# DerryHub/BEVFormer_tensorrt

Hardware: AMD Instinct MI355X
Metric: frames/sec BEVFormer-base bs=1 fp16 end-to-end on MI355X (re-hosted model, random weights, synthetic 6-camera frames) (higher is better)
Workload: dtype f16

## Files before the change

bevformer_tensorrt_amd/csrc/mdconv.h:

```cpp
#ifndef BEVOPS_MDCONV_H_
#define BEVOPS_MDCONV_H_
#include <type_traits>

#include "common.h"

namespace bevops {
enum DcnPath {
  kDcnAuto = 0,
  kDcnLds,
  kDcnStaged,
  kDcnGemm
};

struct DcnVariant {
  int id;
  DcnPath f16, s8;
  int f16_threads;
  bool no_tail, wide;
};
extern thread_local DcnVariant g_dcn_variant;

namespace {

typedef _Float16 f16x8 __attribute__((ext_vector_type(8)));
typedef float f32x16 __attribute__((ext_vector_type(16)));

struct ConvDims {
  int B, Cin, H, W, Cout, Kh, Kw, sh, sw, ph, pw, dh, dw, G, DG, Ho, Wo;
};

template <typename T> __device__ __forceinline__ float tof(T v);
template <> __device__ __forceinline__ float tof<float>(float v) { return v; }
template <> __device__ __forceinline__ float tof<__half>(__half v) { return __half2float(v); }
template <typename T> __device__ __forceinline__ T fromf(float v);
template <> __device__ __forceinline__ float fromf<float>(float v) { return v; }
template <> __device__ __forceinline__ __half fromf<__half>(float v) { return __float2half_rn(v); }

template <typename T>
__global__ __launch_bounds__(256) void nchw_to_nhwc_kernel(const T *__restrict__ in,
                                                           T *__restrict__ out, int C, int HW, int flip = 0) {
  __shared__ T tile[32][33];
  const int b = blockIdx.z;
  const int p0 = blockIdx.x * 32, c0 = blockIdx.y * 32;
  const int tx = threadIdx.x & 31, ty = threadIdx.x >> 5;
  const T *ib = in + (size_t)b * C * HW;
  T *ob = out + (size_t)b * C * HW;
#pragma unroll
  for (int r = 0; r < 32; r += 8) {
    const int c = c0 + ty + r, p = p0 + tx;
    if (c < C && p < HW) {
      if constexpr (sizeof(T) == 1) tile[ty + r][tx] = (T)(ib[(size_t)c * HW + p] ^ (T)flip);
      else tile[ty + r][tx] = ib[(size_t)c * HW + p];
    }
  }
  __syncthreads();
#pragma unroll
  for (int r = 0; r < 32; r += 8) {
    const int p = p0 + ty + r, c = c0 + tx;
    if (c < C && p < HW) ob[(size_t)p * C + c] = tile[tx][ty + r];
  }
}

template <typename T>
__global__ __launch_bounds__(256) void repack_weight_kernel(const T *__restrict__ w,
                                                            T *__restrict__ wt, int Cout,
                                                            int cin_g, int KK, int row_stride) {
  const size_t i = (size_t)blockIdx.x * 256 + threadIdx.x;
  const size_t total = (size_t)Cout * cin_g * KK;
  if (i >= total) return;
  const int ci = (int)(i % cin_g);
  const int t = (int)((i / cin_g) % KK);
  const size_t co = i / ((size_t)cin_g * KK);
  wt[co * row_stride + (size_t)t * cin_g + ci] = w[(co * cin_g + ci) * KK + t];
}

constexpr int kBM = 128, kBN = 128, kBK = 32, kLd = kBK + 8;

struct GemmEpi {
  int HoWo, Cout, co0;
};

constexpr int kFM = 256, kFN = 64, kFK = 64, kFLd = kFK + 8;

constexpr int kGA = kFM * kFK * 2;
template <int WN> struct Glds {
  static constexpr int kN = 32 * WN;
  static constexpr int kThreads = 256 * WN;
  static constexpr int kB = kN * kFK * 2;
  static constexpr int kLds = 2 * (kGA + kB);
  static constexpr int kPieces = 32 / (4 * WN);
};

typedef unsigned u32x4_t __attribute__((ext_vector_type(4)));
__device__ __forceinline__ unsigned swz8(unsigned r) { return (r ^ (r >> 3)) & 7u; }

struct TailPlan {
  int tail_tiles, split, main_tiles;
  float *partial;
  int out_nhwc, relu;
  int om_channels;
};

inline size_t align256(size_t x) { return (x + 255) & ~size_t(255); }

inline bool make_dims(ConvDims &d, int B, int Cin, int H, int W, int Cout, int Kh, int Kw, int sh, int sw,
               int ph, int pw, int dh, int dw, int G, int DG) {
  if (B <= 0 || Cin <= 0 || H <= 0 || W <= 0 || Cout <= 0 || Kh <= 0 || Kw <= 0 || sh <= 0 ||
      sw <= 0 || ph < 0 || pw < 0 || dh <= 0 || dw <= 0 || G <= 0 || DG <= 0)
    return false;
  if (Cin % G || Cout % G || Cin % DG) return false;
  const int Ho = (H + 2 * ph - (dh * (Kh - 1) + 1)) / sh + 1;
  const int Wo = (W + 2 * pw - (dw * (Kw - 1) + 1)) / sw + 1;
  if (Ho <= 0 || Wo <= 0) return false;
  d = ConvDims{B, Cin, H, W, Cout, Kh, Kw, sh, sw, ph, pw, dh, dw, G, DG, Ho, Wo};
  return true;
}

struct WsLayout {
  size_t xt, wt, col, total;
};
inline size_t kpad(const ConvDims &d, size_t es) {
  const size_t kg = (size_t)(d.Cin / d.G) * d.Kh * d.Kw;
  return es == 1 ? ((kg + 15) & ~size_t(15)) : kg;
}
inline WsLayout ws_layout(const ConvDims &d, size_t es) {
  WsLayout w;
  const size_t kp = kpad(d, es);
  w.xt = 0;
  w.wt = align256((size_t)d.B * d.Cin * d.H * d.W * es);
  w.col = w.wt + align256((size_t)d.Cout * kp * es);
  w.total = w.col + align256((size_t)d.B * d.Ho * d.Wo * d.G * kp * es);
  return w;
}

struct DcnCall {
  ConvDims d;
  int dtype;
  const void *input, *offset, *mask, *weight, *bias;
  void *output;
  bool packed;
  bool nhwc;
  bool relu;
  bool exact;
  int om_channels;
  float s_in, s_off, s_mask, s_w, s_out;
  void *workspace;
  size_t workspace_bytes;
  hipStream_t stream;
};

inline DcnCall dcn_call(int dtype, const void *input, const void *offset, const void *mask, const void *weight,
                        const void *bias, void *output, void *workspace, size_t workspace_bytes, int B, int Cin, int H,
                        int W, int Cout, int Kh, int Kw, int sh, int sw, int ph, int pw, int dh, int dw, int G, int DG,
                        void *stream) {
  DcnCall c{};
  (void)make_dims(c.d, B, Cin, H, W, Cout, Kh, Kw, sh, sw, ph, pw, dh, dw, G, DG);
  c.dtype = dtype;
  c.input = input, c.offset = offset, c.mask = mask, c.weight = weight, c.bias = bias, c.output = output;
  c.workspace = workspace, c.workspace_bytes = workspace_bytes;
  c.stream = static_cast<hipStream_t>(stream);
  return c;
}

struct DcnTail {
  int tiles, split;
};
inline DcnTail plan_tail(int blocks, int grid_y, int KK, int slots, size_t room, size_t block_bytes) {
  if (blocks <= slots || grid_y != 1) return DcnTail{0, 1};
  const int left = blocks % slots;
  int split = 0;
  for (int f = KK; f >= 2; --f)
    if (KK % f == 0 && left * f <= slots) { split = f; break; }
  if (left > 0 && left * 2 <= slots && split >= 2 && room >= (size_t)split * left * block_bytes) return DcnTail{left, split};
  return DcnTail{0, 1};
}

enum DcnCopy { kDcnCopyNone, kDcnCopyGeneric, kDcnCopyQuad };
struct DcnPlan {
  DcnPath path;
  int threads;
  int WN;
  DcnTail tail;
  char *partial;
  DcnCopy copy;
  bool repack;
  bool zero_pad;
};
typedef int (*DcnCusFn)();
typedef int (*DcnSlotsFn)(const DcnCall &c, int wn);

inline bool one_deform_group(const ConvDims &d, int g) {
  const int cin_g = d.Cin / d.G, cin_dg = d.Cin / d.DG;
  return cin_g <= cin_dg && (g * cin_g) / cin_dg == (g * cin_g + cin_g - 1) / cin_dg;
}
inline bool one_deform_group(const ConvDims &d) {
  for (int g = 0; g < d.G; ++g)
    if (!one_deform_group(d, g)) return false;
  return true;
}

inline int device_cus() {
  int dev = 0, cus = 0;
  if (hipGetDevice(&dev) != hipSuccess ||
      hipDeviceGetAttribute(&cus, hipDeviceAttributeMultiprocessorCount, dev) != hipSuccess)
    return 0;
  return cus;
}

template <auto Kern>
int resident_blocks(int threads, int lds) {
  static thread_local int cached_dev = -1, cached = 0;
  int dev = 0;
  if (hipGetDevice(&dev) != hipSuccess) return 0;
  if (dev == cached_dev) return cached;
  int per_cu = 0;
  const int cus = device_cus();
  if (cus <= 0 ||
      hipFuncSetAttribute(reinterpret_cast<const void *>(Kern), hipFuncAttributeMaxDynamicSharedMemorySize, lds) != hipSuccess ||
      hipOccupancyMaxActiveBlocksPerMultiprocessor(&per_cu, Kern, threads, lds) != hipSuccess)
    return 0;
  cached_dev = dev;
  cached = per_cu * cus;
  return cached;
}

}
}
#endif
```

bevformer_tensorrt_amd/csrc/mdconv.hip:

```cpp
#include <type_traits>

#include "mdconv.h"

namespace bevops {
constexpr DcnVariant kDcnVariants[] = {
    {0, kDcnAuto, kDcnAuto, 0, false, false},
    {1, kDcnGemm, kDcnAuto, 0, false, false},
    {2, kDcnStaged, kDcnAuto, 256, false, false},
    {3, kDcnStaged, kDcnAuto, 512, false, false},
    {4, kDcnAuto, kDcnAuto, 0, true, false},
    {5, kDcnAuto, kDcnAuto, 0, false, true},
    {6, kDcnStaged, kDcnGemm, 512, false, false},
    {8, kDcnStaged, kDcnStaged, 512, false, false},
    {9, kDcnStaged, kDcnLds, 512, false, false},
};
thread_local DcnVariant g_dcn_variant = kDcnVariants[0];
namespace {

__global__ __launch_bounds__(256) void nchw_to_nhwc_f16q_kernel(const __half *__restrict__ in, __half *__restrict__ out,
                                                                int C, int HW) {
  constexpr int kRow = 128 + 16;
  __shared__ __attribute__((aligned(16))) unsigned char tile[128 * kRow];
  const int b = blockIdx.z;
  const int p0 = blockIdx.x * 128, c0 = blockIdx.y * 64;
  const __half *ib = in + (size_t)b * C * HW;
  __half *ob = out + (size_t)b * C * HW;
#pragma unroll
  for (int it = 0; it < 2; ++it) {
    const int v = threadIdx.x + it * 256;
    const int pq = v & 31, cq = v >> 5;
    const int p = p0 + pq * 4, c = c0 + cq * 4;
    uint2 r[4];
#pragma unroll
    for (int k = 0; k < 4; ++k) r[k] = make_uint2(0u, 0u);
    if (p < HW && c < C) {
#pragma unroll
      for (int k = 0; k < 4; ++k) r[k] = *reinterpret_cast<const uint2 *>(ib + (size_t)(c + k) * HW + p);
    }
    uint2 o[4];
    o[0] = make_uint2(__builtin_amdgcn_perm(r[1].x, r[0].x, 0x05040100u), __builtin_amdgcn_perm(r[3].x, r[2].x, 0x05040100u));
    o[1] = make_uint2(__builtin_amdgcn_perm(r[1].x, r[0].x, 0x07060302u), __builtin_amdgcn_perm(r[3].x, r[2].x, 0x07060302u));
    o[2] = make_uint2(__builtin_amdgcn_perm(r[1].y, r[0].y, 0x05040100u), __builtin_amdgcn_perm(r[3].y, r[2].y, 0x05040100u));
    o[3] = make_uint2(__builtin_amdgcn_perm(r[1].y, r[0].y, 0x07060302u), __builtin_amdgcn_perm(r[3].y, r[2].y, 0x07060302u));
#pragma unroll
    for (int j = 0; j < 4; ++j) *reinterpret_cast<uint2 *>(&tile[(pq * 4 + j) * kRow + cq * 8]) = o[j];
  }
  __syncthreads();
#pragma unroll
  for (int it = 0; it < 4; ++it) {
    const int v = threadIdx.x + it * 256;
    const int ch = v & 7, pl = v >> 3;
    if (p0 + pl < HW && c0 + ch * 8 < C)
      *reinterpret_cast<uint4 *>(ob + (size_t)(p0 + pl) * C + c0 + ch * 8) =
          *reinterpret_cast<const uint4 *>(&tile[pl * kRow + ch * 16]);
  }
}

template <typename T, int V>
__global__ __launch_bounds__(256) void im2col_nhwc_kernel(const T *__restrict__ xt,
                                                          const T *__restrict__ offset,
                                                          const T *__restrict__ mask,
                                                          T *__restrict__ col, ConvDims d) {
  const int vec_per_pix = d.Cin / V;
  const int KK = d.Kh * d.Kw;
  const size_t idx = (size_t)blockIdx.x * 256 + threadIdx.x;
  const int cv = (int)(idx % vec_per_pix);
  const size_t r = idx / vec_per_pix;
  const int t = (int)(r % KK);
  const size_t n = r / KK;
  const int HoWo = d.Ho * d.Wo;
  const size_t N = (size_t)d.B * HoWo;
  if (n >= N) return;
  const int b = (int)(n / HoWo);
  const int pix = (int)(n - (size_t)b * HoWo);
  const int ho = pix / d.Wo, wo = pix - ho * d.Wo;
  const int c = cv * V;
  const int dg = c / (d.Cin / d.DG);
  const int i = t / d.Kw, j = t - i * d.Kw;
  const size_t obase = (((size_t)b * d.DG + dg) * 2 * KK) * HoWo + pix;
  const float off_h = tof(offset[obase + (size_t)(2 * t) * HoWo]);
  const float off_w = tof(offset[obase + (size_t)(2 * t + 1) * HoWo]);
  const float m = tof(mask[(((size_t)b * d.DG + dg) * KK + t) * HoWo + pix]);
  float h_im, w_im;
  {
#pragma clang fp contract(off)
    h_im = (float)(ho * d.sh - d.ph + i * d.dh) + off_h;
    w_im = (float)(wo * d.sw - d.pw + j * d.dw) + off_w;
  }
  float acc[V];
#pragma unroll
  for (int k = 0; k < V; ++k) acc[k] = 0.f;
  if (h_im > -1.f && w_im > -1.f && h_im < (float)d.H && w_im < (float)d.W) {
#pragma clang fp contract(off)
    const float hf = floorf(h_im), wf = floorf(w_im);
    const int h0 = (int)hf, w0 = (int)wf;
    const float lh = h_im - hf, lw = w_im - wf, hh = 1.f - lh, hw = 1.f - lw;
    const float wt[4] = {hh * hw, hh * lw, lh * hw, lh * lw};
// ... 328 lines not shown
      bl[v].x = pk_mul(rb[0][v].x, fw[0]); bl[v].y = pk_mul(rb[0][v].y, fw[0]);
      bl[v].z = pk_mul(rb[0][v].z, fw[0]); bl[v].w = pk_mul(rb[0][v].w, fw[0]);
#pragma unroll
      for (int q = 1; q < 4; ++q) {
        bl[v].x = pk_fma(rb[q][v].x, fw[q], bl[v].x); bl[v].y = pk_fma(rb[q][v].y, fw[q], bl[v].y);
        bl[v].z = pk_fma(rb[q][v].z, fw[q], bl[v].z); bl[v].w = pk_fma(rb[q][v].w, fw[q], bl[v].w);
      }
    }
    __syncthreads();
#pragma unroll
    for (int i = 0; i < NA; ++i) *reinterpret_cast<uint4 *>(&As[ar + RPP * i][ac]) = ra[i];
#pragma unroll
    for (int v = 0; v < NB; ++v) *reinterpret_cast<uint4 *>(&Bs[tid / LPP][cq * 8 * NB + 8 * v]) = bl[v];
    __syncthreads();
    if (step + 1 < nsteps) prefetch(step + 1);
#pragma unroll
    for (int ks = 0; ks < 4; ++ks) {
      const int kk = ks * 16 + (lane >> 5) * 8;
      f16x8 a[2], b[NJ];
#pragma unroll
      for (int i = 0; i < 2; ++i)
        a[i] = *reinterpret_cast<const f16x8 *>(&As[wm * 64 + i * 32 + (lane & 31)][kk]);
#pragma unroll
      for (int j = 0; j < NJ; ++j)
        b[j] = *reinterpret_cast<const f16x8 *>(&Bs[wn * (kFN / WN) + j * 32 + (lane & 31)][kk]);
#pragma unroll
      for (int i = 0; i < 2; ++i)
#pragma unroll
        for (int j = 0; j < NJ; ++j)
          acc[i][j] = __builtin_amdgcn_mfma_f32_32x32x16_f16(a[i], b[j], acc[i][j], 0, 0, 0);
    }
  }
#pragma unroll
  for (int j = 0; j < NJ; ++j) {
    const int n = n0 + wn * (kFN / WN) + j * 32 + (lane & 31);
    if (n >= N) continue;
    const int b = n / HoWo, pix = n - b * HoWo;
    __half *ob = out + ((size_t)b * d.Cout + g * cout_g) * HoWo + pix;
#pragma unroll
    for (int i = 0; i < 2; ++i)
#pragma unroll
      for (int r = 0; r < 16; ++r) {
        const int m = m0 + wm * 64 + i * 32 + (r & 3) + 8 * (r >> 2) + 4 * (lane >> 5);
        if (m < cout_g) {
          float v = acc[i][j][r];
          if (bias) v += __half2float(bias[g * cout_g + m]);
          ob[(size_t)m * HoWo] = __float2half_rn(v);
        }
      }
  }
}


__device__ __forceinline__ void dcn_store4(__half *__restrict__ out, const __half *__restrict__ bias,
                                           const float (&v)[4], int b, int pix, int m, int g,
                                           int cout_g, int Cout, int HoWo, const TailPlan &tp) {
  float o[4];
#pragma unroll
  for (int e = 0; e < 4; ++e) {
    o[e] = v[e];
    if (bias && m + e < cout_g) o[e] += __half2float(bias[g * cout_g + m + e]);
    if (tp.relu) o[e] = fmaxf(o[e], 0.f);
  }
  if (tp.out_nhwc) {
    __half *p = out + ((size_t)b * HoWo + pix) * Cout + g * cout_g + m;
    if (m + 3 < cout_g && (((g * cout_g + m) | Cout) & 3) == 0) {
      uint2 w;
      w.x = pack_h2(o[0], o[1]);
      w.y = pack_h2(o[2], o[3]);
      *reinterpret_cast<uint2 *>(p) = w;
    } else {
#pragma unroll
      for (int e = 0; e < 4; ++e)
        if (m + e < cout_g) p[e] = __float2half_rn(o[e]);
    }
  } else {
    __half *p = out + ((size_t)b * Cout + g * cout_g + m) * HoWo + pix;
#pragma unroll
    for (int e = 0; e < 4; ++e)
      if (m + e < cout_g) p[(size_t)e * HoWo] = __float2half_rn(o[e]);
  }
}

template <int WN>
__global__ __launch_bounds__(256 * WN, WN == 2 ? 2 : 1) void dcn_glds_f16_kernel(
    const __half *__restrict__ xt, const __half *__restrict__ offset,
    const __half *__restrict__ mask, const __half *__restrict__ wt,
    const __half *__restrict__ bias, __half *__restrict__ out, ConvDims d, int g, TailPlan tp) {
  extern __shared__ __attribute__((aligned(16))) char smem[];
  const int tid = threadIdx.x, lane = tid & 63, wave = tid >> 6;
  const int wm = wave & 3, wn = wave >> 2;
  const int KK = d.Kh * d.Kw, cin_g = d.Cin / d.G, cout_g = d.Cout / d.G;
  const int HoWo = d.Ho * d.Wo;
  const int N = d.B * HoWo;
  const int n_tail_blocks = tp.tail_tiles * tp.split;
  const bool is_tail = (int)blockIdx.x < n_tail_blocks;
  int ntile, part = 0;
  if (is_tail) {
    ntile = tp.main_tiles + (int)blockIdx.x / tp.split;
    part = (int)blockIdx.x % tp.split;
  } else {
    ntile = (int)xcd_remap(blockIdx.x - n_tail_blocks, tp.main_tiles);
  }
  constexpr int kN = Glds<WN>::kN, kGB = Glds<WN>::kB, kTh = Glds<WN>::kThreads, kPc = Glds<WN>::kPieces;
  const int n0 = ntile * kN, m0 = blockIdx.y * kFM;
  const int Kg = KK * cin_g;
  const __half *A = wt + (size_t)g * cout_g * Kg;
  const int dg = (g * cin_g) / (d.Cin / d.DG);

  const int pp = tid >> 3, cq = tid & 7;
  const int pn = n0 + pp;
  const bool pvalid = pn < N;
  const int pb = pvalid ? pn / HoWo : 0;
  const int ppix = pvalid ? pn - pb * HoWo : 0;
  const int pho = ppix / d.Wo, pwo = ppix - pho * d.Wo;
  const __amdgpu_buffer_rsrc_t rs_x = __builtin_amdgcn_make_buffer_rsrc(
      const_cast<__half *>(xt), 0, (unsigned)((size_t)d.B * d.H * d.W * d.Cin * 2), 0x00020000);
  const __amdgpu_buffer_rsrc_t rs_w = __builtin_amdgcn_make_buffer_rsrc(
      const_cast<__half *>(A), 0, (unsigned)((size_t)cout_g * Kg * 2), 0x00020000);
  const unsigned ximg_off = (unsigned)(((size_t)pb * d.H * d.W * d.Cin + g * cin_g + cq * 8) * 2);
  const unsigned b_dst = (unsigned)(pp * 128 + ((cq ^ swz8(pp)) << 4));
  constexpr int kPcS = 2 * kPc;
  unsigned a_off[kPcS];
#pragma unroll
  for (int j = 0; j < kPcS; ++j) {
    const unsigned row = (unsigned)((wave * kPcS + j) * 8 + (lane >> 3));
    const unsigned chunk = (lane & 7u) ^ swz8(row);
    a_off[j] = (m0 + (int)row) < cout_g ? (unsigned)(((size_t)(m0 + row) * Kg) * 2 + chunk * 16) : 0xFFFFFFF0u;
  }
  unsigned fa[2], fb;
#pragma unroll
  for (int i = 0; i < 2; ++i) fa[i] = (unsigned)(wm * 64 + i * 32 + (lane & 31));
  fb = (unsigned)(wn * 32 + (lane & 31));
  const unsigned hi = lane >> 5;

  f32x16 acc[2];
#pragma unroll
  for (int i = 0; i < 2; ++i)
#pragma unroll
    for (int r = 0; r < 16; ++r) acc[i][r] = 0.f;

  const int chunks = cin_g / kFK;
  const size_t ob = (((size_t)pb * d.DG + dg) * 2 * KK) * HoWo + ppix;
  const size_t mb = (((size_t)pb * d.DG + dg) * KK) * HoWo + ppix;
  const size_t omb = ((size_t)pb * HoWo + ppix) * (size_t)tp.om_channels + (size_t)dg * 3 * KK;
  auto load_om = [&](int tap, __half &oh, __half &ow, __half &mm) {
    if (tp.om_channels) {
      const unsigned o2 = *reinterpret_cast<const unsigned *>(offset + omb + 2 * tap);
      oh = __ushort_as_half((unsigned short)(o2 & 0xffffu));
      ow = __ushort_as_half((unsigned short)(o2 >> 16));
      mm = offset[omb + 2 * KK + tap];
    } else {
      oh = offset[ob + (size_t)(2 * tap) * HoWo];
      ow = offset[ob + (size_t)(2 * tap + 1) * HoWo];
      mm = mask[mb + (size_t)tap * HoWo];
    }
  };
  const int taps_per_part = is_tail ? KK / tp.split : KK;
  const bool stagger = (size_t)cout_g * Kg * 2 <= (size_t)(2 << 20);
  const int tap_begin = is_tail ? part * taps_per_part : (stagger ? ntile % KK : 0);
  const int n_my_steps = taps_per_part * chunks;
  __half n_oh, n_ow, n_mm;
  load_om(tap_begin, n_oh, n_ow, n_mm);
  int fidx[4];
  unsigned fw[4];
  uint4 rb[4];
  auto footprint = [&](int tap) {
    const float off_h = __half2float(n_oh), off_w = __half2float(n_ow);
    const float m = tp.om_channels ? __half2float(__float2half_rn(1.f / (1.f + __expf(-__half2float(n_mm))))) : __half2float(n_mm);
    load_om(tap + 1 < KK ? tap + 1 : 0, n_oh, n_ow, n_mm);
    const int i = tap / d.Kw, j = tap - i * d.Kw;
    const float h_im = (float)(pho * d.sh - d.ph + i * d.dh) + off_h;
    const float w_im = (float)(pwo * d.sw - d.pw + j * d.dw) + off_w;
    const bool in = pvalid && h_im > -1.f && w_im > -1.f && h_im < (float)d.H && w_im < (float)d.W;
    const float hf = floorf(h_im), wf = floorf(w_im);
    const int h0 = (int)hf, w0 = (int)wf;
    const float lh = h_im - hf, lw = w_im - wf, hh = 1.f - lh, hw = 1.f - lw;
    const float wq[4] = {hh * hw, hh * lw, lh * hw, lh * lw};
    const int hs[4] = {h0, h0, h0 + 1, h0 + 1}, ws[4] = {w0, w0 + 1, w0, w0 + 1};
#pragma unroll
    for (int q = 0; q < 4; ++q) {
      const bool ok = in && hs[q] >= 0 && hs[q] <= d.H - 1 && ws[q] >= 0 && ws[q] <= d.W - 1;
      fidx[q] = ok ? (int)(ximg_off + (unsigned)(hs[q] * d.W + ws[q]) * (unsigned)(d.Cin * 2)) : (int)kDcnSkipOff;
      const float w = ok ? wq[q] * m : 0.f;
      fw[q] = pack_h2(w, w);
    }
  };
  typedef __attribute__((address_space(3))) void lds_void;
  int g_tap = tap_begin, g_chunk = 0, w_tap = tap_begin, w_chunk = 0;
  unsigned c_fw[4] = {0u, 0u, 0u, 0u};
  auto gather_next = [&]() {
    if (g_chunk == 0) footprint(g_tap);
    const int c0 = g_chunk * kFK;
#pragma unroll
    for (int q = 0; q < 4; ++q) {
      rb[q] = __builtin_bit_cast(uint4, __builtin_amdgcn_raw_buffer_load_b128(rs_x, fidx[q], c0 * 2, 0));
      c_fw[q] = fw[q];
    }
    if (++g_chunk == chunks) { g_chunk = 0; g_tap = g_tap + 1 < KK ? g_tap + 1 : 0; }
  };
  auto weights_next = [&](int buf) {
    const int a_s = (w_tap * cin_g + w_chunk * kFK) * 2;
    char *adst = smem + buf * kGA + wave * (kPcS * 1024);
#pragma unroll
    for (int j = 0; j < kPcS; ++j)
      __builtin_amdgcn_raw_ptr_buffer_load_lds(rs_w, (lds_void *)(adst + j * 1024), 16, (int)a_off[j], a_s, 0, 0);
    if (++w_chunk == chunks) { w_chunk = 0; w_tap = w_tap + 1 < KK ? w_tap + 1 : 0; }
  };
  typedef __attribute__((address_space(3))) char lds_char;
  const unsigned b_lds = (unsigned)(size_t)((lds_char *)smem) + (unsigned)(2 * kGA) + b_dst;
  auto blend_store = [&](int buf) {
    u32x4_t bl;
    bl.x = pk_mul(rb[0].x, c_fw[0]); bl.y = pk_mul(rb[0].y, c_fw[0]);
    bl.z = pk_mul(rb[0].z, c_fw[0]); bl.w = pk_mul(rb[0].w, c_fw[0]);
#pragma unroll
    for (int q = 1; q < 4; ++q) {
      bl.x = pk_fma(rb[q].x, c_fw[q], bl.x); bl.y = pk_fma(rb[q].y, c_fw[q], bl.y);
      bl.z = pk_fma(rb[q].z, c_fw[q], bl.z); bl.w = pk_fma(rb[q].w, c_fw[q], bl.w);
    }
    asm volatile("ds_write_b128 %0, %1" ::"v"(b_lds + (unsigned)(buf * kGB)), "v"(bl) : "memory");
  };

  gather_next();
  blend_store(0);
  __builtin_amdgcn_sched_barrier(0);
  if (__builtin_amdgcn_readfirstlane(wave) < kTh / 128) weights_next(0);
  if (n_my_steps > 1) gather_next();
  if (n_my_steps > 1) asm volatile("s_waitcnt vmcnt(4) lgkmcnt(0)" ::: "memory");
  else asm volatile("s_waitcnt vmcnt(0) lgkmcnt(0)" ::: "memory");
  __builtin_amdgcn_s_barrier();

  auto mfma_step = [&](int buf) {
    const char *Ab = smem + buf * kGA;
    const char *Bb = smem + 2 * kGA + buf * kGB;
#pragma unroll
    for (int ks = 0; ks < 4; ++ks) {
      const unsigned c = 2u * ks + hi;
      f16x8 a[2], b;
#pragma unroll
      for (int i = 0; i < 2; ++i)
        a[i] = *reinterpret_cast<const f16x8 *>(Ab + fa[i] * 128 + ((c ^ swz8(fa[i])) << 4));
      b = *reinterpret_cast<const f16x8 *>(Bb + fb * 128 + ((c ^ swz8(fb)) << 4));
#pragma unroll
      for (int i = 0; i < 2; ++i) acc[i] = __builtin_amdgcn_mfma_f32_32x32x16_f16(a[i], b, acc[i], 0, 0, 0);
    }
  };
  const bool upper = __builtin_amdgcn_readfirstlane(wave) >= kTh / 128;
  for (int step = 0; step < n_my_steps; ++step) {
    const bool more1 = step + 1 < n_my_steps, more2 = step + 2 < n_my_steps;
    if (!upper && more1) blend_store((step + 1) & 1);
    __builtin_amdgcn_sched_barrier(0);
    if (!upper && more1) weights_next((step + 1) & 1);
    if (!upper && more2) gather_next();
    __builtin_amdgcn_sched_barrier(0);
    mfma_step(step & 1);
    __builtin_amdgcn_sched_barrier(0);
    if (upper && more1) blend_store((step + 1) & 1);
    __builtin_amdgcn_sched_barrier(0);
    if (upper && more2) gather_next();
    __builtin_amdgcn_sched_barrier(0);
    if (more2) asm volatile("s_waitcnt vmcnt(4) lgkmcnt(0)" ::: "memory");
    else asm volatile("s_waitcnt vmcnt(0) lgkmcnt(0)" ::: "memory");
    __builtin_amdgcn_s_barrier();
  }
  if (is_tail) {
    float4 *pp = reinterpret_cast<float4 *>(tp.partial) +
                 ((((size_t)part * tp.tail_tiles + (ntile - tp.main_tiles)) * gridDim.y + blockIdx.y) * 8) * kTh + tid;
#pragma unroll
    for (int i = 0; i < 2; ++i)
#pragma unroll
      for (int r = 0; r < 4; ++r)
        pp[(i * 4 + r) * kTh] = make_float4(acc[i][4 * r], acc[i][4 * r + 1], acc[i][4 * r + 2], acc[i][4 * r + 3]);
    return;
  }
  {
    const int n = n0 + wn * 32 + (lane & 31);
    if (n < N) {
      const int b = n / HoWo, pix = n - b * HoWo;
#pragma unroll
      for (int i = 0; i < 2; ++i)
#pragma unroll
        for (int rq = 0; rq < 4; ++rq) {
          const int m = m0 + wm * 64 + i * 32 + 8 * rq + 4 * (lane >> 5);
          const float v[4] = {acc[i][4 * rq], acc[i][4 * rq + 1], acc[i][4 * rq + 2], acc[i][4 * rq + 3]};
          dcn_store4(out, bias, v, b, pix, m, g, cout_g, d.Cout, HoWo, tp);
        }
    }
  }
}


template <int WN>
__global__ __launch_bounds__(256 * WN) void dcn_tail_finish_kernel(const __half *__restrict__ bias,
                                                              __half *__restrict__ out, ConvDims d,
                                                              int g, TailPlan tp) {
  const int tid = threadIdx.x, lane = tid & 63, wave = tid >> 6;
  const int wm = wave & 3, wn = wave >> 2;
  const int cout_g = d.Cout / d.G, HoWo = d.Ho * d.Wo, N = d.B * HoWo;
  const int ntile = tp.main_tiles + blockIdx.x;
  constexpr int kTh = Glds<WN>::kThreads;
  const int n0 = ntile * Glds<WN>::kN, m0 = blockIdx.y * kFM;
  const int quad = blockIdx.z, i = quad >> 2, rq = quad & 3;
  float4 a = make_float4(0.f, 0.f, 0.f, 0.f);
  for (int part = 0; part < tp.split; ++part) {
    const float4 v = reinterpret_cast<const float4 *>(tp.partial)[
        ((((size_t)part * tp.tail_tiles + blockIdx.x) * gridDim.y + blockIdx.y) * 8 + quad) * kTh + tid];
    a.x += v.x; a.y += v.y; a.z += v.z; a.w += v.w;
  }
  const int n = n0 + wn * 32 + (lane & 31);
  if (n >= N) return;
  const int b = n / HoWo, pix = n - b * HoWo;
  const float av[4] = {a.x, a.y, a.z, a.w};
  dcn_store4(out, bias, av, b, pix, m0 + wm * 64 + i * 32 + 8 * rq + 4 * (lane >> 5), g, cout_g, d.Cout, HoWo, tp);
}


int lds_f16_slots(const DcnCall &, int wn) {
  return wn == 4 ? resident_blocks<dcn_glds_f16_kernel<4>>(Glds<4>::kThreads, Glds<4>::kLds)
                 : resident_blocks<dcn_glds_f16_kernel<2>>(Glds<2>::kThreads, Glds<2>::kLds);
}

int plan_fp(const DcnCall &c, const DcnVariant &v, DcnCusFn cus, DcnSlotsFn slots, DcnPlan &p) {
  const ConvDims &d = c.d;
  const size_t es = c.dtype == BEVOPS_F32 ? 4 : 2;
  const int HW = d.H * d.W, KK = d.Kh * d.Kw, cin_g = d.Cin / d.G, cout_g = d.Cout / d.G;
  const size_t N = (size_t)d.B * d.Ho * d.Wo;
  if (N > 0x7FFFFFFFull || (size_t)d.B * d.Cin * HW > 0x7FFFFFFF00ull) return BEVOPS_NOT_SUPPORTED;
  const bool fits32 = (size_t)d.B * d.Cin * HW * 2 < 0xFFFFFF00ull && (size_t)d.Cout * cin_g * KK * 2 < 0xFFFFFF00ull;
  p = DcnPlan{};
  p.copy = c.nhwc ? kDcnCopyNone
                  : (es == 2 && HW % 4 == 0 && d.Cin % 8 == 0 && aligned16(c.input) ? kDcnCopyQuad : kDcnCopyGeneric);
  p.repack = !c.packed;
  const bool extras = c.nhwc || c.relu || c.om_channels;
  if (es == 2 && v.f16 != kDcnGemm && fits32 && cin_g % kFK == 0 && (d.Cin / d.DG) % kFK == 0) {
    p.path = kDcnStaged;
    p.threads = v.f16 == kDcnStaged ? v.f16_threads : 512;
    for (int g = 0; g < d.G; ++g) {
      const bool lds = v.f16 == kDcnAuto && one_deform_group(d, g);
      if (extras && !lds) return BEVOPS_NOT_SUPPORTED;
      if (!lds || p.path == kDcnLds) continue;
      const int n_cus = cus();
      if (n_cus <= 0) return BEVOPS_FAILURE;
      const size_t wide_blocks = ((N + Glds<4>::kN - 1) / Glds<4>::kN) * ((cout_g + kFM - 1) / kFM);
      p.WN = v.wide || (!v.no_tail && wide_blocks * 2 >= (size_t)n_cus) ? 4 : 2;
      const int n_slots = slots(c, p.WN);
      if (n_slots <= 0) return BEVOPS_FAILURE;
      const WsLayout w = ws_layout(d, es);
      const int grid_x = (int)((N + 32 * p.WN - 1) / (32 * p.WN)), grid_y = (cout_g + kFM - 1) / kFM;
      p.tail = v.no_tail ? DcnTail{0, 1}
                         : plan_tail(grid_x * grid_y, grid_y, KK, n_slots, w.total - w.col, (size_t)256 * p.WN * 32 * sizeof(float));
      p.partial = static_cast<char *>(c.workspace) + w.col;
      p.path = kDcnLds;
    }
    return BEVOPS_SUCCESS;
  }
  if (extras) return BEVOPS_NOT_SUPPORTED;
  p.path = kDcnGemm;
  const int V = es == 2 ? 8 : 4;
  const bool vec = cin_g % V == 0 && (d.Cin / d.DG) % V == 0;
  if ((N * KK * (d.Cin / (vec ? V : 1)) + 255) / 256 > 0x7FFFFFFFull) return BEVOPS_NOT_SUPPORTED;
  if (es == 2 && (KK * cin_g) % 8 != 0 && ((size_t)cout_g * N + 255) / 256 > 0x7FFFFFFFull) return BEVOPS_NOT_SUPPORTED;
  return BEVOPS_SUCCESS;
}

template <int WN>
int launch_lds_f16(const DcnCall &c, const DcnPlan &p, int g, const __half *xt, const __half *wt) {
  const ConvDims &d = c.d;
  const size_t N = (size_t)d.B * d.Ho * d.Wo;
  const dim3 grid((unsigned)((N + Glds<WN>::kN - 1) / Glds<WN>::kN), (d.Cout / d.G + kFM - 1) / kFM);
  const TailPlan tp{p.tail.tiles, p.tail.split, (int)grid.x - p.tail.tiles,
                    p.tail.tiles ? reinterpret_cast<float *>(p.partial) : nullptr, c.nhwc ? 1 : 0, c.relu ? 1 : 0,
                    c.om_channels};
  hipLaunchKernelGGL(dcn_glds_f16_kernel<WN>, dim3((unsigned)(tp.tail_tiles * tp.split + tp.main_tiles), grid.y),
                     dim3(Glds<WN>::kThreads), Glds<WN>::kLds, c.stream, xt, (const __half *)c.offset,
                     (const __half *)c.mask, wt, (const __half *)c.bias, (__half *)c.output, d, g, tp);
  if (tp.tail_tiles)
    hipLaunchKernelGGL(dcn_tail_finish_kernel<WN>, dim3((unsigned)tp.tail_tiles, grid.y, 8), dim3(Glds<WN>::kThreads), 0,
                       c.stream, (const __half *)c.bias, (__half *)c.output, d, g, tp);
  return launch_status();
}

template <typename T>
int launch_fp(const DcnCall &c, const DcnPlan &p) {
  const ConvDims &d = c.d;
  hipStream_t st = c.stream;
  const WsLayout w = ws_layout(d, sizeof(T));
  char *ws = static_cast<char *>(c.workspace);
  T *xt = reinterpret_cast<T *>(ws + w.xt);
  T *wt = reinterpret_cast<T *>(ws + w.wt);
  T *col = reinterpret_cast<T *>(ws + w.col);
  const int HW = d.H * d.W, KK = d.Kh * d.Kw, cin_g = d.Cin / d.G, cout_g = d.Cout / d.G;
  const size_t N = (size_t)d.B * d.Ho * d.Wo;
  if (p.copy == kDcnCopyNone)
    xt = const_cast<T *>(static_cast<const T *>(c.input));
  else if (p.copy == kDcnCopyQuad)
    hipLaunchKernelGGL(nchw_to_nhwc_f16q_kernel, dim3((HW + 127) / 128, (d.Cin + 63) / 64, d.B), dim3(256), 0, st,
                       (const __half *)c.input, (__half *)xt, d.Cin, HW);
  else
    hipLaunchKernelGGL((nchw_to_nhwc_kernel<T>), dim3((HW + 31) / 32, (d.Cin + 31) / 32, d.B), dim3(256),
                       0, st, (const T *)c.input, xt, d.Cin, HW);
  const size_t wtot = (size_t)d.Cout * cin_g * KK;
  if (!p.repack)
    wt = const_cast<T *>(static_cast<const T *>(c.weight));
  else
    hipLaunchKernelGGL((repack_weight_kernel<T>), dim3((unsigned)((wtot + 255) / 256)), dim3(256), 0, st,
                       (const T *)c.weight, wt, d.Cout, cin_g, KK, KK * cin_g);
  if constexpr (sizeof(T) == 2) {
    if (p.path != kDcnGemm) {
      const dim3 grid((unsigned)((N + kFN - 1) / kFN), (cout_g + kFM - 1) / kFM);
      for (int g = 0; g < d.G; ++g) {
        if (p.path == kDcnLds && one_deform_group(d, g)) {
          const int rc = p.WN == 4 ? launch_lds_f16<4>(c, p, g, (const __half *)xt, (const __half *)wt)
                                   : launch_lds_f16<2>(c, p, g, (const __half *)xt, (const __half *)wt);
          if (rc != BEVOPS_SUCCESS) return rc;
        } else {
          auto staged = p.threads == 256 ? dcn_fused_f16_kernel<256> : dcn_fused_f16_kernel<512>;
          hipLaunchKernelGGL(staged, grid, dim3(p.threads), 0, st, (const __half *)xt, (const __half *)c.offset,
                             (const __half *)c.mask, (const __half *)wt, (const __half *)c.bias, (__half *)c.output, d, g);
        }
      }
      return launch_status();
    }
  }
  constexpr int VMAX = sizeof(T) == 2 ? 8 : 4;
  const bool vec = cin_g % VMAX == 0 && (d.Cin / d.DG) % VMAX == 0;
  const size_t blocks = (N * KK * (d.Cin / (vec ? VMAX : 1)) + 255) / 256;
  auto im2col = vec ? im2col_nhwc_kernel<T, VMAX> : im2col_nhwc_kernel<T, 1>;
  hipLaunchKernelGGL(im2col, dim3((unsigned)blocks), dim3(256), 0, st, xt, (const T *)c.offset, (const T *)c.mask, col, d);
  const int Kg = KK * cin_g;
  for (int g = 0; g < d.G; ++g) {
    const GemmEpi e{d.Ho * d.Wo, d.Cout, g * cout_g};
    const T *Ag = wt + (size_t)g * cout_g * Kg;
    const T *Bg = col + (size_t)g * N * Kg;
    if constexpr (sizeof(T) == 2) {
      if (Kg % 8 == 0)
        hipLaunchKernelGGL(gemm_tn_f16_kernel, dim3((unsigned)((N + kBN - 1) / kBN), (cout_g + kBM - 1) / kBM),
                           dim3(256), 0, st, (const __half *)Ag, (const __half *)Bg, (const __half *)c.bias,
                           (__half *)c.output, cout_g, (int)N, Kg, e);
      else
        hipLaunchKernelGGL(gemm_tn_f16_ragged_kernel, dim3((unsigned)(((size_t)cout_g * N + 255) / 256)), dim3(256), 0,
                           st, (const __half *)Ag, (const __half *)Bg, (const __half *)c.bias, (__half *)c.output,
                           cout_g, (int)N, Kg, e);
    } else {
      hipLaunchKernelGGL(gemm_tn_f32_kernel, dim3((unsigned)((N + 63) / 64), (cout_g + 63) / 64), dim3(256),
                         0, st, (const float *)Ag, (const float *)Bg, (const float *)c.bias, (float *)c.output,
                         cout_g, (int)N, Kg, e);
    }
  }
  return launch_status();
}

int forward_fp(const DcnCall &c) {
  if (!c.input || !c.offset || (!c.mask && !c.om_channels) || !c.weight || !c.output || !c.workspace) return BEVOPS_BAD_PARAM;
  const ConvDims &d = c.d;
  if (d.B == 0) return BEVOPS_BAD_PARAM;
  if (c.om_channels && (c.om_channels < d.DG * 3 * d.Kh * d.Kw || (c.om_channels & 1))) return BEVOPS_BAD_PARAM;
  if (c.dtype != BEVOPS_F32 && c.dtype != BEVOPS_F16) return BEVOPS_NOT_SUPPORTED;
// ... 109 lines not shown
```

Baseline: 103.5.

## Precompute DCN bilinear footprint table in LDS and stage NHWC epilogue through LDS rows

In the wide (WN=4) LDS deformable-conv kernel, every block now computes all taps' bilinear sample indices and weights once up front and keeps them in a per-tap LDS table, instead of recomputing them in the gather loop. The gather loop then reads the table with ds_read_b128. A second change stages the NHWC epilogue outputs through an LDS row image so the global stores become coalesced 16-byte writes. The cost is extra LDS per block (the table), which can lower occupancy, plus a prologue sync. New variants are added to choose between the skeleton modes.

```diff
diff --git a/bevformer_tensorrt_amd/csrc/mdconv.h b/bevformer_tensorrt_amd/csrc/mdconv.h
--- a/bevformer_tensorrt_amd/csrc/mdconv.h
+++ b/bevformer_tensorrt_amd/csrc/mdconv.h
@@ -12,11 +12,17 @@
   kDcnGemm
 };
 
+enum DcnSkeleton {
+  kDcnSkelFull = 0,
+  kDcnSkelParent,
+  kDcnSkelTable
+};
 struct DcnVariant {
   int id;
   DcnPath f16, s8;
   int f16_threads;
   bool no_tail, wide;
+  DcnSkeleton skel;
 };
 extern thread_local DcnVariant g_dcn_variant;
 
@@ -91,6 +97,11 @@
   static constexpr int kPieces = 32 / (4 * WN);
 };
 
+constexpr int kDcnTabTap = 2 * Glds<4>::kN * 16;
+constexpr int kDcnTabTaps = (160 * 1024 - Glds<4>::kLds) / kDcnTabTap;
+constexpr int kDcnEpiRow = kFM * 2 + 16;
+static_assert(Glds<4>::kN * kDcnEpiRow <= Glds<4>::kLds && Glds<2>::kN * kDcnEpiRow <= Glds<2>::kLds, "epilogue image");
+
 typedef unsigned u32x4_t __attribute__((ext_vector_type(4)));
 __device__ __forceinline__ unsigned swz8(unsigned r) { return (r ^ (r >> 3)) & 7u; }
 
@@ -99,6 +110,7 @@
   float *partial;
   int out_nhwc, relu;
   int om_channels;
+  int row_store;
 };
 
 inline size_t align256(size_t x) { return (x + 255) & ~size_t(255); }
@@ -185,6 +197,8 @@
   DcnCopy copy;
   bool repack;
   bool zero_pad;
+  bool table;
+  bool row_store;
 };
 typedef int (*DcnCusFn)();
 typedef int (*DcnSlotsFn)(const DcnCall &c, int wn);
diff --git a/bevformer_tensorrt_amd/csrc/mdconv.hip b/bevformer_tensorrt_amd/csrc/mdconv.hip
--- a/bevformer_tensorrt_amd/csrc/mdconv.hip
+++ b/bevformer_tensorrt_amd/csrc/mdconv.hip
@@ -4,15 +4,21 @@
 
 namespace bevops {
 constexpr DcnVariant kDcnVariants[] = {
-    {0, kDcnAuto, kDcnAuto, 0, false, false},
-    {1, kDcnGemm, kDcnAuto, 0, false, false},
-    {2, kDcnStaged, kDcnAuto, 256, false, false},
-    {3, kDcnStaged, kDcnAuto, 512, false, false},
-    {4, kDcnAuto, kDcnAuto, 0, true, false},
-    {5, kDcnAuto, kDcnAuto, 0, false, true},
-    {6, kDcnStaged, kDcnGemm, 512, false, false},
-    {8, kDcnStaged, kDcnStaged, 512, false, false},
-    {9, kDcnStaged, kDcnLds, 512, false, false},
+    {0, kDcnAuto, kDcnAuto, 0, false, false, kDcnSkelFull},
+    {1, kDcnGemm, kDcnAuto, 0, false, false, kDcnSkelFull},
+    {2, kDcnStaged, kDcnAuto, 256, false, false, kDcnSkelFull},
+    {3, kDcnStaged, kDcnAuto, 512, false, false, kDcnSkelFull},
+    {4, kDcnAuto, kDcnAuto, 0, true, false, kDcnSkelFull},
+    {5, kDcnAuto, kDcnAuto, 0, false, true, kDcnSkelFull},
+    {6, kDcnStaged, kDcnGemm, 512, false, false, kDcnSkelFull},
+    {8, kDcnStaged, kDcnStaged, 512, false, false, kDcnSkelFull},
+    {9, kDcnStaged, kDcnLds, 512, false, false, kDcnSkelFull},
+    {10, kDcnAuto, kDcnAuto, 0, false, false, kDcnSkelParent},
+    {14, kDcnAuto, kDcnAuto, 0, true, false, kDcnSkelParent},
+    {15, kDcnAuto, kDcnAuto, 0, false, true, kDcnSkelParent},
+    {20, kDcnAuto, kDcnAuto, 0, false, false, kDcnSkelTable},
+    {24, kDcnAuto, kDcnAuto, 0, true, false, kDcnSkelTable},
+    {25, kDcnAuto, kDcnAuto, 0, false, true, kDcnSkelTable},
 };
 thread_local DcnVariant g_dcn_variant = kDcnVariants[0];
 namespace {
@@ -507,11 +513,34 @@
   }
 }
 
-template <int WN>
+__device__ __forceinline__ void dcn_footprint(const ConvDims &d, bool pvalid, int pho, int pwo, unsigned img_off, int tap,
+                                              float off_h, float off_w, float m, unsigned skip, int (&fidx)[4],
+                                              unsigned (&fw)[4]) {
+  const int i = tap / d.Kw, j = tap - i * d.Kw;
+  const float h_im = (float)(pho * d.sh - d.ph + i * d.dh) + off_h;
+  const float w_im = (float)(pwo * d.sw - d.pw + j * d.dw) + off_w;
+  const bool in = pvalid && h_im > -1.f && w_im > -1.f && h_im < (float)d.H && w_im < (float)d.W;
+  const float hf = floorf(h_im), wf = floorf(w_im);
+  const int h0 = (int)hf, w0 = (int)wf;
+  const float lh = h_im - hf, lw = w_im - wf, hh = 1.f - lh, hw = 1.f - lw;
+  const float wq[4] = {hh * hw, hh * lw, lh * hw, lh * lw};
+  const int hs[4] = {h0, h0, h0 + 1, h0 + 1}, ws[4] = {w0, w0 + 1, w0, w0 + 1};
+#pragma unroll
+  for (int q = 0; q < 4; ++q) {
+    const bool ok = in && hs[q] >= 0 && hs[q] <= d.H - 1 && ws[q] >= 0 && ws[q] <= d.W - 1;
+    fidx[q] = ok ? (int)(img_off + (unsigned)(hs[q] * d.W + ws[q]) * (unsigned)(d.Cin * 2)) : (int)skip;
+    const float w = ok ? wq[q] * m : 0.f;
+    fw[q] = pack_h2(w, w);
+  }
+}
+constexpr unsigned kDcnSkipTab = 0xFFFFFF00u;
+
+template <int WN, bool TAB>
 __global__ __launch_bounds__(256 * WN, WN == 2 ? 2 : 1) void dcn_glds_f16_kernel(
     const __half *__restrict__ xt, const __half *__restrict__ offset,
     const __half *__restrict__ mask, const __half *__restrict__ wt,
     const __half *__restrict__ bias, __half *__restrict__ out, ConvDims d, int g, TailPlan tp) {
+  static_assert(!TAB || WN == 4, "the footprint table needs the LDS a second 64-pixel block would take");
   extern __shared__ __attribute__((aligned(16))) char smem[];
   const int tid = threadIdx.x, lane = tid & 63, wave = tid >> 6;
   const int wm = wave & 3, wn = wave >> 2;
@@ -585,37 +614,43 @@
   const bool stagger = (size_t)cout_g * Kg * 2 <= (size_t)(2 << 20);
   const int tap_begin = is_tail ? part * taps_per_part : (stagger ? ntile % KK : 0);
   const int n_my_steps = taps_per_part * chunks;
+  auto mask_value = [&](__half mm) {
+    return tp.om_channels ? __half2float(__float2half_rn(1.f / (1.f + __expf(-__half2float(mm))))) : __half2float(mm);
+  };
   __half n_oh, n_ow, n_mm;
-  load_om(tap_begin, n_oh, n_ow, n_mm);
+  if constexpr (!TAB) load_om(tap_begin, n_oh, n_ow, n_mm);
   int fidx[4];
   unsigned fw[4];
   uint4 rb[4];
   auto footprint = [&](int tap) {
     const float off_h = __half2float(n_oh), off_w = __half2float(n_ow);
-    const float m = tp.om_channels ? __half2float(__float2half_rn(1.f / (1.f + __expf(-__half2float(n_mm))))) : __half2float(n_mm);
+    const float m = mask_value(n_mm);
     load_om(tap + 1 < KK ? tap + 1 : 0, n_oh, n_ow, n_mm);
-    const int i = tap / d.Kw, j = tap - i * d.Kw;
-    const float h_im = (float)(pho * d.sh - d.ph + i * d.dh) + off_h;
-    const float w_im = (float)(pwo * d.sw - d.pw + j * d.dw) + off_w;
-    const bool in = pvalid && h_im > -1.f && w_im > -1.f && h_im < (float)d.H && w_im < (float)d.W;
-    const float hf = floorf(h_im), wf = floorf(w_im);
-    const int h0 = (int)hf, w0 = (int)wf;
-    const float lh = h_im - hf, lw = w_im - wf, hh = 1.f - lh, hw = 1.f - lw;
-    const float wq[4] = {hh * hw, hh * lw, lh * hw, lh * lw};
-    const int hs[4] = {h0, h0, h0 + 1, h0 + 1}, ws[4] = {w0, w0 + 1, w0, w0 + 1};
-#pragma unroll
-    for (int q = 0; q < 4; ++q) {
-      const bool ok = in && hs[q] >= 0 && hs[q] <= d.H - 1 && ws[q] >= 0 && ws[q] <= d.W - 1;
-      fidx[q] = ok ? (int)(ximg_off + (unsigned)(hs[q] * d.W + ws[q]) * (unsigned)(d.Cin * 2)) : (int)kDcnSkipOff;
-      const float w = ok ? wq[q] * m : 0.f;
-      fw[q] = pack_h2(w, w);
-    }
+    dcn_footprint(d, pvalid, pho, pwo, ximg_off, tap, off_h, off_w, m, kDcnSkipOff, fidx, fw);
   };
   typedef __attribute__((address_space(3))) void lds_void;
+  typedef __attribute__((address_space(3))) char lds_char;
+  const int tab_tap0 = is_tail ? tap_begin : 0;
+  const unsigned tab_lds = (unsigned)(size_t)((lds_char *)smem) + (unsigned)Glds<WN>::kLds + (unsigned)(pp * 16);
   int g_tap = tap_begin, g_chunk = 0, w_tap = tap_begin, w_chunk = 0;
   unsigned c_fw[4] = {0u, 0u, 0u, 0u};
   auto gather_next = [&]() {
-    if (g_chunk == 0) footprint(g_tap);
+    if constexpr (TAB) {
+      if (g_chunk == 0) {
+        u32x4_t ri, rw;
+        asm volatile("ds_read_b128 %0, %2\n\tds_read_b128 %1, %2 offset:%3\n\ts_waitcnt lgkmcnt(0)"
+                     : "=&v"(ri), "=&v"(rw)
+                     : "v"(tab_lds + (unsigned)((g_tap - tab_tap0) * kDcnTabTap)), "n"(kDcnTabTap / 2)
+                     : "memory");
+#pragma unroll
+        for (int q = 0; q < 4; ++q) {
+          fidx[q] = (int)(ri[q] + (unsigned)(cq * 16));
+          fw[q] = rw[q];
+        }
+      }
+    } else {
+      if (g_chunk == 0) footprint(g_tap);
+    }
     const int c0 = g_chunk * kFK;
 #pragma unroll
     for (int q = 0; q < 4; ++q) {
@@ -632,7 +667,6 @@
       __builtin_amdgcn_raw_ptr_buffer_load_lds(rs_w, (lds_void *)(adst + j * 1024), 16, (int)a_off[j], a_s, 0, 0);
     if (++w_chunk == chunks) { w_chunk = 0; w_tap = w_tap + 1 < KK ? w_tap + 1 : 0; }
   };
-  typedef __attribute__((address_space(3))) char lds_char;
   const unsigned b_lds = (unsigned)(size_t)((lds_char *)smem) + (unsigned)(2 * kGA) + b_dst;
   auto blend_store = [&](int buf) {
     u32x4_t bl;
@@ -646,10 +680,46 @@
     asm volatile("ds_write_b128 %0, %1" ::"v"(b_lds + (unsigned)(buf * kGB)), "v"(bl) : "memory");
   };
 
-  gather_next();
-  blend_store(0);
-  __builtin_amdgcn_sched_barrier(0);
-  if (__builtin_amdgcn_readfirstlane(wave) < kTh / 128) weights_next(0);
+  if constexpr (TAB) {
+    if (__builtin_amdgcn_readfirstlane(wave) < kTh / 128) weights_next(0);
+    for (int r = tid; r < taps_per_part * kN; r += kTh) {
+      const int t = r / kN, p = r - t * kN, tap = tab_tap0 + t;
+      const int rn = n0 + p;
+      const bool rvalid = rn < N;
+      const int rb_ = rvalid ? rn / HoWo : 0;
+      const int rpix = rvalid ? rn - rb_ * HoWo : 0;
+      const int rho = rpix / d.Wo, rwo = rpix - rho * d.Wo;
+      __half oh, ow, mm;
+      if (tp.om_channels) {
+        const size_t o = ((size_t)rb_ * HoWo + rpix) * (size_t)tp.om_channels + (size_t)dg * 3 * KK;
+        const unsigned o2 = *reinterpret_cast<const unsigned *>(offset + o + 2 * tap);
+        oh = __ushort_as_half((unsigned short)(o2 & 0xffffu));
+        ow = __ushort_as_half((unsigned short)(o2 >> 16));
+        mm = offset[o + 2 * KK + tap];
+      } else {
+        const size_t o = (((size_t)rb_ * d.DG + dg) * 2 * KK) * HoWo + rpix;
+        oh = offset[o + (size_t)(2 * tap) * HoWo];
+        ow = offset[o + (size_t)(2 * tap + 1) * HoWo];
+        mm = mask[(((size_t)rb_ * d.DG + dg) * KK) * HoWo + rpix + (size_t)tap * HoWo];
+      }
+      int ri[4];
+      unsigned rw[4];
+      dcn_footprint(d, rvalid, rho, rwo, (unsigned)(((size_t)rb_ * d.H * d.W * d.Cin + g * cin_g) * 2), tap,
+                    __half2float(oh), __half2float(ow), mask_value(mm), kDcnSkipTab, ri, rw);
+      char *rec = smem + Glds<WN>::kLds + t * kDcnTabTap + p * 16;
+      *reinterpret_cast<uint4 *>(rec) = make_uint4((unsigned)ri[0], (unsigned)ri[1], (unsigned)ri[2], (unsigned)ri[3]);
+      *reinterpret_cast<uint4 *>(rec + kDcnTabTap / 2) = make_uint4(rw[0], rw[1], rw[2], rw[3]);
+    }
+    __syncthreads();
+    gather_next();
+    blend_store(0);
+    __builtin_amdgcn_sched_barrier(0);
+  } else {
+    gather_next();
+    blend_store(0);
+    __builtin_amdgcn_sched_barrier(0);
+    if (__builtin_amdgcn_readfirstlane(wave) < kTh / 128) weights_next(0);
+  }
   if (n_my_steps > 1) gather_next();
   if (n_my_steps > 1) asm volatile("s_waitcnt vmcnt(4) lgkmcnt(0)" ::: "memory");
   else asm volatile("s_waitcnt vmcnt(0) lgkmcnt(0)" ::: "memory");
@@ -698,6 +768,34 @@
         pp[(i * 4 + r) * kTh] = make_float4(acc[i][4 * r], acc[i][4 * r + 1], acc[i][4 * r + 2], acc[i][4 * r + 3]);
     return;
   }
+  if (tp.row_store) {
+    char *row = smem + (wn * 32 + (lane & 31)) * kDcnEpiRow;
+#pragma unroll
+    for (int i = 0; i < 2; ++i)
+#pragma unroll
+      for (int rq = 0; rq < 4; ++rq) {
+        const int ml = wm * 64 + i * 32 + 8 * rq + 4 * (lane >> 5), m = m0 + ml;
+        float o[4];
+#pragma unroll
+        for (int e = 0; e < 4; ++e) {
+          o[e] = acc[i][4 * rq + e];
+          if (bias && m + e < cout_g) o[e] += __half2float(bias[g * cout_g + m + e]);
+          if (tp.relu) o[e] = fmaxf(o[e], 0.f);
+        }
+        *reinterpret_cast<uint2 *>(row + ml * 2) = make_uint2(pack_h2(o[0], o[1]), pack_h2(o[2], o[3]));
+      }
+    __syncthreads();
+    const int pieces = (cout_g - m0 < kFM ? cout_g - m0 : kFM) / 8;
+    __half *ob = out + g * cout_g + m0;
+    for (int r = tid; r < kN * (kFM / 8); r += kTh) {
+      const int p = r / (kFM / 8), pc = r % (kFM / 8);
+      const int n = n0 + p;
+      if (n < N && pc < pieces)
+        *reinterpret_cast<uint4 *>(ob + (size_t)n * d.Cout + pc * 8) =
+            *reinterpret_cast<const uint4 *>(smem + p * kDcnEpiRow + pc * 16);
+    }
+    return;
+  }
   {
     const int n = n0 + wn * 32 + (lane & 31);
     if (n < N) {
@@ -741,8 +839,10 @@
 
 
 int lds_f16_slots(const DcnCall &, int wn) {
-  return wn == 4 ? resident_blocks<dcn_glds_f16_kernel<4>>(Glds<4>::kThreads, Glds<4>::kLds)
-                 : resident_blocks<dcn_glds_f16_kernel<2>>(Glds<2>::kThreads, Glds<2>::kLds);
+  if (wn != 4) return resident_blocks<dcn_glds_f16_kernel<2, false>>(Glds<2>::kThreads, Glds<2>::kLds);
+  const int plain = resident_blocks<dcn_glds_f16_kernel<4, false>>(Glds<4>::kThreads, Glds<4>::kLds);
+  const int table = resident_blocks<dcn_glds_f16_kernel<4, true>>(Glds<4>::kThreads, Glds<4>::kLds + kDcnTabTaps * kDcnTabTap);
+  return plain < table ? plain : table;
 }
 
 int plan_fp(const DcnCall &c, const DcnVariant &v, DcnCusFn cus, DcnSlotsFn slots, DcnPlan &p) {
@@ -775,6 +875,8 @@
       p.tail = v.no_tail ? DcnTail{0, 1}
                          : plan_tail(grid_x * grid_y, grid_y, KK, n_slots, w.total - w.col, (size_t)256 * p.WN * 32 * sizeof(float));
       p.partial = static_cast<char *>(c.workspace) + w.col;
+      p.table = v.skel != kDcnSkelParent && p.WN == 4 && KK <= kDcnTabTaps;
+      p.row_store = v.skel == kDcnSkelFull && c.nhwc && cout_g % 8 == 0 && aligned16(c.output);
       p.path = kDcnLds;
     }
     return BEVOPS_SUCCESS;
@@ -795,9 +897,17 @@
   const dim3 grid((unsigned)((N + Glds<WN>::kN - 1) / Glds<WN>::kN), (d.Cout / d.G + kFM - 1) / kFM);
   const TailPlan tp{p.tail.tiles, p.tail.split, (int)grid.x - p.tail.tiles,
                     p.tail.tiles ? reinterpret_cast<float *>(p.partial) : nullptr, c.nhwc ? 1 : 0, c.relu ? 1 : 0,
-                    c.om_channels};
-  hipLaunchKernelGGL(dcn_glds_f16_kernel<WN>, dim3((unsigned)(tp.tail_tiles * tp.split + tp.main_tiles), grid.y),
-                     dim3(Glds<WN>::kThreads), Glds<WN>::kLds, c.stream, xt, (const __half *)c.offset,
+                    c.om_channels, p.row_store ? 1 : 0};
+  auto kern = dcn_glds_f16_kernel<WN, false>;
+  int lds = Glds<WN>::kLds;
+  if constexpr (WN == 4) {
+    if (p.table) {
+      kern = dcn_glds_f16_kernel<4, true>;
+      lds += d.Kh * d.Kw * kDcnTabTap;
+    }
+  }
+  hipLaunchKernelGGL(kern, dim3((unsigned)(tp.tail_tiles * tp.split + tp.main_tiles), grid.y),
+                     dim3(Glds<WN>::kThreads), lds, c.stream, xt, (const __half *)c.offset,
                      (const __half *)c.mask, wt, (const __half *)c.bias, (__half *)c.output, d, g, tp);
   if (tp.tail_tiles)
     hipLaunchKernelGGL(dcn_tail_finish_kernel<WN>, dim3((unsigned)tp.tail_tiles, grid.y, 8), dim3(Glds<WN>::kThreads), 0,
```

New measurement: 106.0 (median of 6 runs). +2.4%, better.
